# Serverless-Federated-Learning/FedLesScan

Hardware: AMD Instinct MI355X
Metric: aggregated GB/s (device-resident) — N-client FedAvg fp32 reduction (higher is better)
Workload: dtype f32

## Files before the change

### fedlesscan_amd/_lib.py

```python
from __future__ import annotations

import ctypes
import os
import re
import sysconfig
import threading

from .aggregator.exceptions import (
    AggregationError,
    InsufficientClientResults,
    InvalidParameterShapeError,
)

PKG = os.path.dirname(os.path.abspath(__file__))
REPO = os.path.dirname(PKG)
LIB_PATH = os.path.join(PKG, "_native", "libfedavg_hip.so")
BENCH_LIB_PATH = os.path.join(PKG, "_native", "libfedavg_hip_bench.so")
HOSTFAST_PATH = os.path.join(PKG, "_native", "_hostfast" + (sysconfig.get_config_var("EXT_SUFFIX") or ".so"))
HEADER = os.path.join(REPO, "include", "fedavg_hip.h")
BENCH_HEADER = os.path.join(REPO, "include", "fedavg_hip_bench.h")
ABI_VERSION = 7

FA_OK, FA_ERR_ARG, FA_ERR_NO_CLIENTS, FA_ERR_SHAPE, FA_ERR_HIP = range(5)

# ... 19 lines not shown
    "fa_finalize_f32": (_int, [_vp, _f32, _vp, _i64, _vp]),
    "fa_fedavg_bf16": (_int, [_vp, _i64, _i64, _i64, _vp, _vp, _f32, _vp, _vp, _vp]),
    "fa_fedavg_f16": (_int, [_vp, _i64, _i64, _i64, _vp, _vp, ctypes.c_uint16, _vp, _vp]),
    "fa_fold_f16": (_int, [_vp, _i64, _i64, _i64, _vp, _vp, _vp, ctypes.c_uint16, _int, _vp, _vp]),
    "fa_fedavg_bf16_ptrs": (_int, [_vp, _i64, _i64, _vp, _vp, _f32, _int, _vp, _vp, _vp]),
    "fa_fedavg_bf16_ptrs_hostf": (_int, [_vp, _i64, _i64, _vp, _vp, _f32, _int, _vp, _vp, _vp]),
    "fa_fedavg_f16_ptrs": (_int, [_vp, _i64, _i64, _vp, _vp, ctypes.c_uint16, _int, _vp, _vp]),
    "fa_rounds_create": (_int, [_vp, _int]),
    "fa_rounds_destroy": (_int, [_vp]),
    "fa_fedavg_f32_rounds": (_int, [_vp, _vp, _i64, _i64, _vp, _vp, _f32, _vp, _int, _vp, _vp, _vp]),
    "fa_fedavg_bf16_rounds": (_int, [_vp, _vp, _i64, _i64, _vp, _vp, _f32, _vp, _vp, _int, _vp, _vp, _vp]),
    "fa_fedavg_f32_rounds_hostf": (_int, [_vp, _vp, _i64, _i64, _vp, _vp, _f32, _vp, _int, _vp, _vp, _vp]),
    "fa_fedavg_bf16_rounds_hostf": (_int, [_vp, _vp, _i64, _i64, _vp, _vp, _f32, _vp, _vp, _int, _vp, _vp, _vp]),
    "fa_rounds_wait": (_int, [_vp, _int, _vp]),
    "fa_rounds_check": (_int, [_vp]),
    "fa_rounds_timeouts": (_int, [_vp]),
    "fa_rounds_form": (ctypes.c_char_p, [_int]),
    "fa_fedavg_f16_rounds": (_int, [_vp, _vp, _i64, _i64, _vp, _vp, ctypes.c_uint16, _vp, _int, _vp, _vp, _vp]),
    "fa_rounds_form_f16": (ctypes.c_char_p, []),
    "fa_fedavg_f64_rounds": (_int, [_vp, _vp, _i64, _i64, _vp, _vp, _f64, _vp, _int, _vp, _vp, _vp]),
    "fa_rounds_form_f64": (ctypes.c_char_p, []),
    "fa_peers_create": (_int, [_vp, _int, _int, _int, _i64]),
    "fa_peers_destroy": (_int, [_vp]),
    "fa_peers_handle_bytes": (_int, []),
    "fa_peers_handle": (_int, [_vp, _vp]),
    "fa_peers_open": (_int, [_vp, _vp]),
    "fa_peers_send": (_vp, [_vp]),
    "fa_peers_rounds": (_vp, [_vp]),
    "fa_peers_exchange": (_int, [_vp, _int, _vp, _vp, _vp, _vp]),
    "fa_fedavg_f64": (_int, [_vp, _i64, _i64, _i64, _vp, _vp, _f64, _vp, _vp]),
    "fa_fold_f64": (_int, [_vp, _i64, _i64, _i64, _vp, _vp, _vp, _f64, _int, _vp, _vp]),
    "fa_fedavg_f64_ptrs": (_int, [_vp, _i64, _i64, _vp, _vp, _f64, _int, _vp, _vp]),
    "fa_layers_plan": (_int, [_vp, _vp, _i64, _int, _i64, _int, _vp, _vp, _vp, _vp]),
    "fa_fedavg_f32_layers": (_int, [_vp, _vp, _i64, _i64, _i64, _int, _vp, _vp, _f32, _vp, _vp]),
    "fa_fedavg_bf16_layers": (_int, [_vp, _vp, _i64, _i64, _i64, _int, _vp, _vp, _f32, _vp, _vp, _vp]),
    "fa_fedavg_f16_layers": (_int, [_vp, _vp, _i64, _i64, _i64, _int, _vp, _vp, ctypes.c_uint16, _vp, _vp]),
    "fa_fedavg_f64_layers": (_int, [_vp, _vp, _i64, _i64, _i64, _int, _vp, _vp, _f64, _vp, _vp]),
    "fa_fedavg_i32": (_int, [_vp, _i64, _i64, _i64, _vp, _f64, _vp, _vp]),
    "fa_fedavg_i64": (_int, [_vp, _i64, _i64, _i64, _vp, _f64, _vp, _vp]),
    "fa_fedavg_i32_ptrs": (_int, [_vp, _i64, _i64, _vp, _vp, _f64, _int, _vp, _vp]),
    "fa_fedavg_i64_ptrs": (_int, [_vp, _i64, _i64, _vp, _vp, _f64, _int, _vp, _vp]),
    "fa_fedavg_i32_layers": (_int, [_vp, _vp, _i64, _i64, _i64, _int, _vp, _vp, _f64, _vp, _vp]),
    "fa_fedavg_i64_layers": (_int, [_vp, _vp, _i64, _i64, _i64, _int, _vp, _vp, _f64, _vp, _vp]),
    "fa_npz_index":(_int, [_vp, _i64, _vp, _vp, _vp, _vp, _vp, _int]),
    "fa_crc32": (_int, [_vp, _i64, ctypes.c_uint32, _int, ctypes.POINTER(ctypes.c_uint32)]),
    "fa_pack": (_int, [_vp, _vp, _vp, _vp, _i64, _int]),
    "fa_bson_elements": (_i64, [_vp, _i64, _i64, _vp, _vp, _vp, _vp, _vp, _vp, _i64]),
    "fa_bson_walk": (_i64, [_vp, _i64, _i64, _vp, _vp, _vp, _vp, _vp, _vp, _vp, _i64]),
    "fa_host_is_pinned": (_int, [_vp, _i64]),
    "fa_host_alloc": (_int, [_vp, _i64]),
    "fa_host_free": (_int, [_vp]),
    "fa_copy_h2d": (_int, [_vp, _vp, _i64, _vp]),
    "fa_copy_peer": (_int, [_vp, _int, _vp, _int, _i64, _vp]),
    "fa_set_autotune": (_int, [_int]),
    "fa_autotune_pending": (_int, []),
    "fa_fold_form": (ctypes.c_char_p, [_int, _i64, _i64, _i64, _int, _vp]),
    "fa_tune_cache_path": (_int, [ctypes.c_char_p]),
    "fa_tune_export": (_i64, [_vp, _i64]),
    "fa_tune_import": (_int, [ctypes.c_char_p]),
    "fa_step_lookup": (_int, [ctypes.c_char_p]),
    "fa_step_record": (_int, [ctypes.c_char_p, _int]),
    "fa_ingest_create": (_int, [_vp, _i64, _i64, _int, _int]),
    "fa_ingest_rows_per_chunk": (_int, [_vp]),
    "fa_ingest_begin": (_int, [_vp, _vp, _vp, _i64]),
    "fa_ingest_add": (_int, [_vp, _vp, _vp, _i64, _f32, _f32, _int]),
    "fa_ingest_finish": (_int, [_vp, _f32]),
# ... 149 lines not shown
```

### fedlesscan_amd/csrc/fedavg.hip

```cpp
#include "fold_kernels.hpp"
#include "peer_exchange.hpp"

#include <mutex>

namespace {

constexpr int kFactorSlots = 8;
struct FactorSlot {
    float* host = nullptr;
    float* dev = nullptr;
    size_t cap = 0;
    hipEvent_t ready = nullptr;
    hipEvent_t done = nullptr;
    bool pending = false;
};
struct FactorRing {
    std::mutex mu;
    FactorSlot slot[kFactorSlots];
    int next = 0;
    hipStream_t stage = nullptr;
};
FactorRing g_factor_rings[16];

constexpr int kFillFloats = 256;
// ... 407 lines not shown
    hipStream_t st = (hipStream_t)stream;
    StreamDevice on_stream_device(stream);
    if (aligned16(X) && aligned16(out) && (ldx % 2 == 0)) {
        if (s)
            hipLaunchKernelGGL((k_fedavg_f64_v2<8, true>), grid_for((P >> 1) + 1), dim3(kBlock), 0, st, X, N, P,
                               ldx, a, s, divisor, out);
        else
            hipLaunchKernelGGL((k_fedavg_f64_v2<8, false>), grid_for((P >> 1) + 1), dim3(kBlock), 0, st, X, N, P,
                               ldx, a, s, divisor, out);
        return check_launch("k_fedavg_f64_v2");
    }
    if (s)
        hipLaunchKernelGGL(k_fedavg_f64<true>, grid_for(P), dim3(kBlock), 0, st, X, N, P, ldx, a, s, divisor,
                           out);
    else
        hipLaunchKernelGGL(k_fedavg_f64<false>, grid_for(P), dim3(kBlock), 0, st, X, N, P, ldx, a, s, divisor,
                           out);
    return check_launch("k_fedavg_f64");
}

int fa_fold_f64(const double* X, int64_t N, int64_t P, int64_t ldx, const double* a, const double* s,
                const double* acc_in, double divisor, int finalize, double* out, void* stream) {
    return f64_fold(X, N, P, ldx, a, s, acc_in, divisor, finalize, out, stream);
}

int fa_fedavg_f64_ptrs(const double* const* xi, int64_t N, int64_t P, const double* a, const double* s,
                       double divisor, int rows_aligned, double* out, void* stream) {
    return f64_rows_fold(xi, N, P, a, s, divisor, rows_aligned, out, stream);
}

int fa_layers_plan(const int64_t* cols, const int32_t* aligned, int64_t L, int unit_lg, int64_t cus, int units,
                   fa_layer_plan* plan, int64_t* tiles, int64_t* elems, int* units_out) {
    return layers_plan(cols, aligned, L, unit_lg, cus, units, plan, tiles, elems, units_out);
}

int fa_fedavg_f32_layers(const float* const* xi, const fa_layer_plan* plan, int64_t L, int64_t N, int64_t tiles,
                         int units, const float* a, const float* s, float divisor, float* out, void* stream) {
    return layers_fold(kLayersF32, "fa_fedavg_f32_layers", (const void* const*)xi, plan, L, N, tiles, units, 0, a, s,
                       (double)divisor, out, nullptr, stream);
}

int fa_fedavg_bf16_layers(const uint16_t* const* xi, const fa_layer_plan* plan, int64_t L, int64_t N, int64_t tiles,
                          int units, const float* a, const float* s, float divisor, float* out_f32,
                          uint16_t* out_bf16, void* stream) {
    return layers_fold(kLayersBf16, "fa_fedavg_bf16_layers", (const void* const*)xi, plan, L, N, tiles, units, 0, a, s,
                       (double)divisor, out_f32, out_bf16, stream);
}

int fa_fedavg_f16_layers(const uint16_t* const* xi, const fa_layer_plan* plan, int64_t L, int64_t N, int64_t tiles,
                         int units, const uint16_t* a, const uint16_t* s, uint16_t divisor, uint16_t* out,
                         void* stream) {
    return layers_fold(kLayersF16, "fa_fedavg_f16_layers", (const void* const*)xi, plan, L, N, tiles, units, 0, a, s,
                       (double)half_bits_to_float(divisor), out, nullptr, stream);
}

int fa_fedavg_f64_layers(const double* const* xi, const fa_layer_plan* plan, int64_t L, int64_t N, int64_t tiles,
                         int units, const double* a, const double* s, double divisor, double* out, void* stream) {
    return layers_fold(kLayersF64, "fa_fedavg_f64_layers", (const void* const*)xi, plan, L, N, tiles, units, 0, a, s,
                       divisor, out, nullptr, stream);
}

int fa_fedavg_i32(const int32_t* X, int64_t N, int64_t P, int64_t ldx, const int64_t* a, double divisor,
                  double* out, void* stream) {
    int rc = check_common(N, P, ldx, X, a, out);
    if (rc) return rc;
    if (P == 0) { g_err[0] = 0; return FA_OK; }
// ... 183 lines not shown
```

### fedlesscan_amd/csrc/fold_kernels.hpp

```cpp
#pragma once
#include <hip/hip_runtime.h>
#include <stdarg.h>
#include <stdint.h>
#include <stdio.h>
#include <stdlib.h>
#include <string.h>

#include <atomic>
#include <map>
#include <mutex>
#include <string>
#include <tuple>
#include <type_traits>
#include <vector>

#include "fedavg_hip.h"
#include "octet_grid.hpp"
#include "layer_plan.hpp"
#include "tuner.hpp"

#pragma clang fp contract(off)

namespace {

// ... 1992 lines not shown
    for (; i < N; ++i) acc = acc + term1<SCORED>(((const gf32*)xi[i])[c], a[i], SCORED ? s[i] : 1.0f);
    return acc / divisor;
}

template <int U, int C, bool SCORED>
__global__ __launch_bounds__(kBlock) void k_fold_f32_layers(
    const float* const* __restrict__ xi, const fa_layer_plan* __restrict__ plan, int64_t L, int64_t N,
    const float* __restrict__ a, const float* __restrict__ s, float divisor, float* __restrict__ out,
    int64_t ntiles) {
    int64_t l = 0;
    for (int64_t bid = blockIdx.x; bid < ntiles; bid += gridDim.x) {
        const LayerTile t = layer_tile(plan, L, bid, l);
        l = t.l;
        const float* const* x = xi + l * N;
        float* o = out + t.offset;
        if (!t.aligned) {
            const int64_t c = t.bid * kBlock + threadIdx.x;
            if (c < t.cols) o[c] = fold_column_f32<SCORED>(x, c, N, a, s, divisor);
            continue;
        }
        f32x4* O4 = reinterpret_cast<f32x4*>(o);
        octet_tile<C, kBlock, 2>(
            t.bid, t.cols,
            [&](int64_t q) { fold_quads_rows<U, C, SCORED, gf32x4>(x, q, N, a, s, divisor, O4 + q); },
            [&](int64_t q) { fold_quads_rows<U, 1, SCORED, gf32x4>(x, q, N, a, s, divisor, O4 + q); },
            [&](int64_t col) {
                for (; col < t.cols; ++col) {
                    float acc = term1<SCORED>(((const gf32*)x[0])[col], a[0], SCORED ? s[0] : 1.0f);
                    for (int64_t i = 1; i < N; ++i)
                        acc = acc + term1<SCORED>(((const gf32*)x[i])[col], a[i], SCORED ? s[i] : 1.0f);
                    o[col] = acc / divisor;
                }
            });
    }
}

template <int U, int C, bool SCORED>
__global__ __launch_bounds__(kBlock) void k_fedavg_bf16_layers(
    const uint16_t* const* __restrict__ xi, const fa_layer_plan* __restrict__ plan, int64_t L, int64_t N,
    const float* __restrict__ a, const float* __restrict__ s, float divisor, float* __restrict__ out,
    uint16_t* __restrict__ outb, int64_t ntiles) {
    int64_t l = 0;
    for (int64_t bid = blockIdx.x; bid < ntiles; bid += gridDim.x) {
        const LayerTile t = layer_tile(plan, L, bid, l);
        l = t.l;
        const uint16_t* const* x = xi + l * N;
        float* o = out ? out + t.offset : nullptr;
        uint16_t* ob = outb ? outb + t.offset : nullptr;
        if (!t.aligned) {
            const int64_t c = t.bid * kBlock + threadIdx.x;
            if (c < t.cols) st_column_bf16(fold_column_bf16<SCORED>(TableRows<gu16>{x, c}, N, a, s, divisor), o, ob, c);
            continue;
        }
        octet_tile<C>(
            t.bid, t.cols,
            [&](int64_t q) { fold_octets<U, C, SCORED>(TableRows<gu32x4>{x, q}, N, a, s, divisor, o, ob, q); },
            [&](int64_t q) { fold_octets<U, 1, SCORED>(TableRows<gu32x4>{x, q}, N, a, s, divisor, o, ob, q); },
            [&](int64_t col) {
                for (; col < t.cols; ++col)
                    st_column_bf16(fold_column_bf16<SCORED>(TableRows<gu16>{x, col}, N, a, s, divisor), o, ob, col);
            });
    }
}

template <class A, int U, int C, bool SCORED>
__device__ __forceinline__ void native_layers(const typename A::E* const* __restrict__ xi,
// ... 1481 lines not shown
    switch (kind) {
        case kLayersF32: {
            const float* const* x = (const float* const*)xi;
            const float *af = (const float*)a, *sf = (const float*)s;
            if (s) FA_LAY(k_fold_f32_layers, true, x, plan, L, N, af, sf, (float)divisor, (float*)out);
            else FA_LAY(k_fold_f32_layers, false, x, plan, L, N, af, sf, (float)divisor, (float*)out);
            break;
        }
        case kLayersBf16: {
            const uint16_t* const* x = (const uint16_t* const*)xi;
            const float *af = (const float*)a, *sf = (const float*)s;
            if (s) FA_LAY(k_fedavg_bf16_layers, true, x, plan, L, N, af, sf, (float)divisor, (float*)out, (uint16_t*)outb);
            else FA_LAY(k_fedavg_bf16_layers, false, x, plan, L, N, af, sf, (float)divisor, (float*)out, (uint16_t*)outb);
            break;
        }
        case kLayersF16: {
            const uint16_t* const* x = (const uint16_t* const*)xi;
            const uint16_t *ah = (const uint16_t*)a, *sh = (const uint16_t*)s;
            if (s) FA_LAY(k_fedavg_f16_layers, true, x, plan, L, N, ah, sh, (float)divisor, (uint16_t*)out);
            else FA_LAY(k_fedavg_f16_layers, false, x, plan, L, N, ah, sh, (float)divisor, (uint16_t*)out);
            break;
        }
        default: {
            const double* const* x = (const double* const*)xi;
            const double *ad = (const double*)a, *sd = (const double*)s;
            if (s) FA_LAY(k_fedavg_f64_layers, true, x, plan, L, N, ad, sd, divisor, (double*)out);
            else FA_LAY(k_fedavg_f64_layers, false, x, plan, L, N, ad, sd, divisor, (double*)out);
            break;
        }
    }
#undef FA_LAY
}

inline int layers_fold(int kind, const char* what, const void* const* xi, const fa_layer_plan* plan, int64_t L,
                       int64_t N, int64_t tiles, int units, int64_t grid_cap, const void* a, const void* s,
                       double divisor, void* out, void* outb, void* stream) {
    if (kind < kLayersF32 || kind > kLayersF64) return fail(FA_ERR_ARG, "%s: unknown dtype %d", what, kind);
    if (L < 0 || N < 0 || tiles < 0)
        return fail(FA_ERR_ARG, "negative size (L=%lld, N=%lld, tiles=%lld)", (long long)L, (long long)N,
                    (long long)tiles);
    if (N == 0) return fail(FA_ERR_NO_CLIENTS, "no client results to aggregate (N == 0)");
    if (units != 1 && units != 2 && units != 4)
        return fail(FA_ERR_ARG, "%s: %d units per lane (1, 2 or 4)", what, units);
    if (grid_cap < 0) return fail(FA_ERR_ARG, "%s: negative grid cap", what);
    if (L == 0 || tiles == 0) { g_err[0] = 0; return FA_OK; }
    const bool any_out = kind == kLayersBf16 ? (out || outb) : out != nullptr;
    if (!xi || !plan || !a || !any_out) return fail(FA_ERR_ARG, "null xi/plan/a/out pointer");
    if (!aligned16(out) || (kind == kLayersBf16 && !aligned16(outb)))
        return fail(FA_ERR_ARG, "%s needs 16-B aligned outputs", what);
    if (tiles > (int64_t)0x7FFFFFFF) return fail(FA_ERR_ARG, "too many tiles for one launch");
    hipStream_t st = (hipStream_t)stream;
    StreamDevice on_stream_device(stream);
    int64_t g = tile_grid(tiles, -1, cu_count());
    if (grid_cap > 0 && g > grid_cap) g = grid_cap;
    if (kind != kLayersBf16) outb = nullptr;
    switch (units) {
        case 4: launch_layers<4>(kind, st, (unsigned)g, xi, plan, L, N, tiles, a, s, divisor, out, outb); break;
        case 2: launch_layers<2>(kind, st, (unsigned)g, xi, plan, L, N, tiles, a, s, divisor, out, outb); break;
        default: launch_layers<1>(kind, st, (unsigned)g, xi, plan, L, N, tiles, a, s, divisor, out, outb); break;
    }
    return check_launch(what);
}

template <class I, int C>
void launch_int_layers(hipStream_t st, unsigned g, const typename I::T* const* xi, const fa_layer_plan* plan,
                       const fa_layer_plan& one, int64_t L, int64_t N, int64_t tiles, const int64_t* a, const double* s,
                       double divisor, double* out) {
    if (s)
        hipLaunchKernelGGL((k_fedavg_int_layers<I, kLayersU, C, true>), dim3(g), dim3(kBlock), 0, st, xi, plan, one, L,
                           N, a, s, divisor, out, tiles);
    else
        hipLaunchKernelGGL((k_fedavg_int_layers<I, kLayersU, C, false>), dim3(g), dim3(kBlock), 0, st, xi, plan, one, L,
                           N, a, s, divisor, out, tiles);
}

template <class I>
void launch_int_layers_units(int units, hipStream_t st, unsigned g, const typename I::T* const* xi,
                             const fa_layer_plan* plan, const fa_layer_plan& one, int64_t L, int64_t N, int64_t tiles,
                             const int64_t* a, const double* s, double divisor, double* out) {
    switch (units) {
        case 4: launch_int_layers<I, 4>(st, g, xi, plan, one, L, N, tiles, a, s, divisor, out); break;
        case 2: launch_int_layers<I, 2>(st, g, xi, plan, one, L, N, tiles, a, s, divisor, out); break;
        default: launch_int_layers<I, 1>(st, g, xi, plan, one, L, N, tiles, a, s, divisor, out); break;
    }
}
// ... 18 lines not shown
    int64_t g = tile_grid(tiles, -1, cu_count());
    if (grid_cap > 0 && g > grid_cap) g = grid_cap;
    launch_int_layers_units<I>(units, st, (unsigned)g, xi, plan, fa_layer_plan{0, 0, 0, 0}, L, N, tiles, a, s, divisor,
                               out);
    return check_launch(what);
}

template <class I>
int int_rows_fold(const char* what, const typename I::T* const* xi, int64_t N, int64_t P, const int64_t* a,
                  const double* s, double divisor, int rows_aligned, double* out, void* stream) {
    int rc = check_common(N, P, P, xi, a, out);
    if (rc) return rc;
    if (P == 0) { g_err[0] = 0; return FA_OK; }
    if (rows_aligned && !aligned16(out))
        return fail(FA_ERR_ARG, "the unit form of the integer row-table fold needs 16-B aligned rows and out");
    hipStream_t st = (hipStream_t)stream;
    StreamDevice on_stream_device(stream);
    const int64_t cus = cu_count();
    const int32_t al = rows_aligned != 0;
    const int units = pick_layer_units(&P, &al, 1, I::LG, cus);
    fa_layer_plan one;
    int64_t elems = 0;
    const int64_t tiles = fill_layer_plan(&P, &al, 1, units, I::LG, &one, &elems);
    if (tiles > (int64_t)0x7FFFFFFF) return fail(FA_ERR_ARG, "too many tiles for one launch");
    launch_int_layers_units<I>(units, st, (unsigned)tile_grid(tiles, -1, cus), xi, nullptr, one, 1, N, tiles, a, s,
                               divisor, out);
    return check_launch(what);
}

inline int layers_plan(const int64_t* cols, const int32_t* aligned, int64_t L, int unit_lg, int64_t cus, int units,
                       fa_layer_plan* plan, int64_t* tiles, int64_t* elems, int* units_out) {
    if (L < 0 || cus < 1 || unit_lg < 1 || unit_lg > 3)
        return fail(FA_ERR_ARG, "fa_layers_plan: L=%lld, cus=%lld, unit_lg=%d", (long long)L, (long long)cus, unit_lg);
    if (units != 0 && units != 1 && units != 2 && units != 4)
        return fail(FA_ERR_ARG, "fa_layers_plan: %d units per lane (0, 1, 2 or 4)", units);
    if (!tiles || !elems || !units_out || (L > 0 && (!cols || !aligned || !plan)))
        return fail(FA_ERR_ARG, "fa_layers_plan: null pointer");
    for (int64_t l = 0; l < L; ++l)
        if (cols[l] < 0) return fail(FA_ERR_ARG, "fa_layers_plan: layer %lld has %lld columns", (long long)l,
                                     (long long)cols[l]);
    if (units == 0) units = pick_layer_units(cols, aligned, L, unit_lg, cus);
    *tiles = fill_layer_plan(cols, aligned, L, units, unit_lg, plan, elems);
    *units_out = units;
    g_err[0] = 0;
    return FA_OK;
}

}
```

### fedlesscan_amd/csrc/layer_plan.hpp

```cpp
#pragma once
#include <stdint.h>

#include "fedavg_hip.h"
#include "octet_grid.hpp"

constexpr int64_t kLayerOutAlign = 64;

inline int64_t layer_tiles(int64_t cols, bool aligned, int units, int unit_lg) {
    if (cols <= 0) return 0;
    if (!aligned) return (cols + kBlock - 1) / kBlock;
    return octet_grid(cols, units, 0, 1, unit_lg).tiles;
}

inline int64_t layers_total_tiles(const int64_t* cols, const int32_t* aligned, int64_t L, int units, int unit_lg) {
    int64_t t = 0;
    for (int64_t l = 0; l < L; ++l) t += layer_tiles(cols[l], aligned[l] != 0, units, unit_lg);
    return t;
}

inline int pick_layer_units(const int64_t* cols, const int32_t* aligned, int64_t L, int unit_lg, int64_t cus) {
    for (int c = 4; c > 1; c >>= 1)
        if (tile_grid(layers_total_tiles(cols, aligned, L, c, unit_lg), -1, cus) * 8 >= cus * 7) return c;
    return 1;
}

inline int64_t fill_layer_plan(const int64_t* cols, const int32_t* aligned, int64_t L, int units, int unit_lg,
                               fa_layer_plan* plan, int64_t* elems) {
    int64_t t = 0, off = 0;
    for (int64_t l = 0; l < L; ++l) {
        plan[l].cols = cols[l];
        plan[l].offset = off;
        plan[l].tile0 = t;
        plan[l].aligned = aligned[l] != 0;
        t += layer_tiles(cols[l], aligned[l] != 0, units, unit_lg);
        off += (cols[l] + kLayerOutAlign - 1) / kLayerOutAlign * kLayerOutAlign;
    }
    *elems = off;
    return t;
}
```

### fedlesscan_amd/engine.py

```python
from __future__ import annotations

import ctypes
import functools
import operator
import os
import threading
from typing import List, NamedTuple, Optional, Sequence

import numpy as np
import torch

from . import _lib
from .aggregator.exceptions import InvalidParameterShapeError

_TORCH_TO_NP = {torch.float32: np.float32, torch.float64: np.float64, torch.int32: np.int32,
                torch.int64: np.int64, torch.float16: np.float16}
_NP_TO_TORCH = {np.dtype(np.float32): torch.float32, np.dtype(np.float64): torch.float64,
                np.dtype(np.int32): torch.int32, np.dtype(np.int64): torch.int64,
                np.dtype(np.float16): torch.float16}
ROW_ALIGN = 64


def default_device() -> torch.device:
    if not torch.cuda.is_available():
# ... 656 lines not shown
        a, s = f.to(dev)
        _lib.call("fa_fedavg_f64_rounds", r, X.data_ptr(), N, ldx, a.data_ptr(), _ptr(s), float(f.div),
                  addr(out), rounds, offs, oo, st)
    else:
        raise InvalidParameterShapeError(
            f"the rounds fold takes float32, bfloat16, float16 or float64 rows, got {X.dtype}")
    return r


def wait_round(state: ctypes.c_void_p, k: int, stream: torch.cuda.Stream) -> None:
    _lib.call("fa_rounds_wait", state, int(k), stream.cuda_stream)


def _equal_stride_view(rows, host_ptrs: np.ndarray, P: int) -> Optional[torch.Tensor]:
    N = len(rows)
    if N < 2 or P == 0:
        return None
    esize = rows[0].element_size()
    step = int(host_ptrs[1] - host_ptrs[0])
    if step < P * esize or step % esize:
        return None
    if (np.diff(host_ptrs) != step).any():
        return None
    base, last = rows[0], rows[-1]
    if last.untyped_storage().data_ptr() != base.untyped_storage().data_ptr():
        return None
    return base.as_strided((N, P), (step // esize, 1))


_dtype_of = operator.attrgetter("dtype")
_ROW_TABLE_DTYPES = (torch.float32, torch.bfloat16, torch.float16, torch.float64, torch.int32, torch.int64)
_INT_ROWS = {torch.int32: "fa_fedavg_i32_ptrs", torch.int64: "fa_fedavg_i64_ptrs"}
_NO_CAPTURE_TABLE = (torch.float64, torch.int32, torch.int64)
stats = {"rows16_folds": 0, "rows64_folds": 0, "stacked_groups": 0, "layer_table_folds": 0, "rows_int_folds": 0}


class RowSet:

    def __init__(self, rows: Sequence[torch.Tensor]):
        rows = list(rows)
        N = len(rows)
        if N == 0:
            _lib.check(_lib.FA_ERR_NO_CLIENTS, "RowSet")
        r0 = rows[0]
        P, dev, dt = r0.numel(), r0.device, r0.dtype
        if not r0.is_cuda:
            raise ValueError("rows must be CUDA (HIP) tensors")
        if (set(map(torch.Tensor.numel, rows)) != {P} or set(map(_dtype_of, rows)) != {dt}
                or not all(map(torch.Tensor.is_contiguous, rows))
                or set(map(torch.Tensor.get_device, rows)) != {r0.get_device()}):
            raise InvalidParameterShapeError("all rows must be contiguous with equal size, dtype, device")
        self.rows = rows
        self.N, self.P, self.device, self.dtype = N, P, dev, dt
        self.view = None
        self.ptrs = None
        self.host_ptrs = None
        self.aligned = False
        if dt in _ROW_TABLE_DTYPES and P > 0 and not (dt in _NO_CAPTURE_TABLE
                                                      and torch.cuda.is_current_stream_capturing()):
            host_ptrs = self.host_ptrs = np.fromiter(map(torch.Tensor.data_ptr, rows), dtype=np.int64, count=N)
            self.view = _equal_stride_view(rows, host_ptrs, P)
            if self.view is None:
                self.ptrs = torch.from_numpy(host_ptrs).to(dev)
                self.aligned = not (host_ptrs % 16).any()

    def overlaps(self, t: torch.Tensor) -> bool:
        if self.host_ptrs is None or self.P == 0 or t.numel() == 0:
# ... 165 lines not shown


_LAYER_TABLE = {
    torch.float32: ("fa_fedavg_f32_layers", 2),
    torch.bfloat16: ("fa_fedavg_bf16_layers", 3),
    torch.float16: ("fa_fedavg_f16_layers", 3),
    torch.float64: ("fa_fedavg_f64_layers", 1),
    torch.int32: ("fa_fedavg_i32_layers", 2),
    torch.int64: ("fa_fedavg_i64_layers", 1),
}
_shape_of = operator.attrgetter("shape")
_cu_counts: dict = {}


def _cus(dev: torch.device) -> int:
    k = dev.index if dev.index is not None else torch.cuda.current_device()
    n = _cu_counts.get(k)
    if n is None:
        n = _cu_counts[k] = int(torch.cuda.get_device_properties(k).multi_processor_count)
    return n


def layer_plan(cols: Sequence[int], aligned: Sequence[bool], unit_lg: int, cus: int, units: int = 0):
    L = len(cols)
    c = np.ascontiguousarray(cols, dtype=np.int64)
    al = np.ascontiguousarray(aligned, dtype=np.int32)
    plan = np.zeros((L, 4), dtype=np.int64)
    tiles, elems, u = ctypes.c_int64(), ctypes.c_int64(), ctypes.c_int()
    _lib.call("fa_layers_plan", c.ctypes.data, al.ctypes.data, L, unit_lg, cus, units, plan.ctypes.data,
              ctypes.addressof(tiles), ctypes.addressof(elems), ctypes.addressof(u))
    return plan, tiles.value, elems.value, u.value


class ModelRowSet:

    def __init__(self, parameters: Sequence[Sequence[torch.Tensor]], layers: Optional[Sequence[int]] = None):
        params = list(parameters)
        N = len(params)
        if N == 0:
            _lib.check(_lib.FA_ERR_NO_CLIENTS, "ModelRowSet")
        lis = list(range(min(map(len, params)))) if layers is None else list(layers)
        cols_of = [list(map(operator.itemgetter(li), params)) for li in lis]
        t0 = cols_of[0][0] if cols_of else None
        if t0 is not None and not (isinstance(t0, torch.Tensor) and t0.is_cuda):
            raise ValueError("layers must be CUDA (HIP) tensors")
        self.N, self.L, self.layers = N, len(lis), lis
        self.device = t0.device if t0 is not None else None
        self.dtype = t0.dtype if t0 is not None else None
        self.shapes, self.sizes = [], []
        host_ptrs = np.zeros((self.L, N), dtype=np.int64)
        for k, col in enumerate(cols_of):
            shp = col[0].shape
            if (set(map(_shape_of, col)) != {shp} or set(map(_dtype_of, col)) != {self.dtype}
                    or not all(map(torch.Tensor.is_contiguous, col))
                    or set(map(torch.Tensor.get_device, col)) != {t0.get_device()}):
                raise InvalidParameterShapeError(
                    f"layer {lis[k]}: all clients' tensors must be contiguous with one shape, dtype and device")
            self.shapes.append(tuple(shp))
            self.sizes.append(col[0].numel())
            host_ptrs[k] = np.fromiter(map(torch.Tensor.data_ptr, col), dtype=np.int64, count=N)
        self.tensors = cols_of
        self.host_ptrs = host_ptrs
        self.esize = t0.element_size() if t0 is not None else 0
        self.entry = None
        self._rowsets: dict = {}
        self.ptrs = self.plan = self.host_plan = None
        self.tiles = self.elems = self.units = 0
        if self.dtype in _LAYER_TABLE and self.L:
            self.entry, lg = _LAYER_TABLE[self.dtype]
            sizes = np.asarray(self.sizes, dtype=np.int64)
            aligned = ~((host_ptrs % 16) != 0).any(axis=1) | (sizes == 0)
            self.host_plan, self.tiles, self.elems, self.units = layer_plan(sizes, aligned, lg, _cus(self.device))
            both = torch.from_numpy(np.concatenate([host_ptrs.reshape(-1), self.host_plan.reshape(-1)])).to(self.device)
            self.ptrs, self.plan = both[:self.L * N], both[self.L * N:]
        self.offsets = [int(o) for o in self.host_plan[:, 1]] if self.host_plan is not None else []

    def overlaps(self, t: torch.Tensor) -> bool:
        if self.L == 0 or t.numel() == 0:
            return False
        lo = t.data_ptr()
        hi = lo + t.numel() * t.element_size()
        nbytes = (np.asarray(self.sizes, dtype=np.int64) * self.esize)[:, None]
        return bool(np.any((self.host_ptrs < hi) & (lo < self.host_ptrs + nbytes)))

    def rowset(self, k: int) -> RowSet:
        rs = self._rowsets.get(k)
        if rs is None:
            rows = [t.reshape(-1) for t in self.tensors[k]]
            if self.ptrs is None or self.sizes[k] == 0:
                rs = RowSet(rows)
            else:
                rs = RowSet.__new__(RowSet)
                rs.rows, rs.N, rs.P, rs.device, rs.dtype = rows, self.N, self.sizes[k], self.device, self.dtype
                rs.view = None
                rs.ptrs = self.ptrs[k * self.N:(k + 1) * self.N]
                rs.host_ptrs = self.host_ptrs[k]
                rs.aligned = bool(self.host_plan[k, 3])
            self._rowsets[k] = rs
        return rs

    def split(self, flat: torch.Tensor) -> List[torch.Tensor]:
        return [flat[o:o + n].reshape(s) for o, n, s in zip(self.offsets, self.sizes, self.shapes)]


def layer_table_enabled() -> bool:
    return os.environ.get("FEDAVG_LAYER_TABLE", "1") != "0"

# ... 18 lines not shown
    if len(weights) != N or (scores is not None and len(scores) != N):
        raise InvalidParameterShapeError(f"{N} clients but {len(weights)} weights"
                                         + ("" if scores is None else f" / {len(scores)} scores"))
    bf16 = ms.dtype == torch.bfloat16
    if (out_bf16 is not None or want_bf16) and not bf16:
        raise InvalidParameterShapeError("want_bf16 / out_bf16 are for bfloat16 layers")
    f = None
    if ms.entry is not None and not torch.cuda.is_current_stream_capturing():
        f = _layer_factors(ms.dtype, weights, scores, total)
    if f is None:
        if out is not None or out_bf16 is not None:
            raise InvalidParameterShapeError("out / out_bf16 need the layer-table route (no promotion, no capture)")
        res = [fold_rows(ms.rowset(k), weights, scores, total=total, want_bf16=want_bf16) for k in range(ms.L)]
        if want_bf16:
            return ([r[0].reshape(s) for r, s in zip(res, ms.shapes)],
                    [r[1].reshape(s) for r, s in zip(res, ms.shapes)])
        return [r.reshape(s) for r, s in zip(res, ms.shapes)]
    dev, E = ms.device, ms.elems
    res_dt = torch.float32 if bf16 else torch.float64 if ms.dtype in _INT_ROWS else ms.dtype
    _check_out("out", out, res_dt, E)
    _check_out("out_bf16", out_bf16, torch.bfloat16, E)

    def usable(t):
        return t is not None and t.data_ptr() % 16 == 0 and not ms.overlaps(t)

    dst, dstb = out, out_bf16
    out = out if usable(out) else None
    outb = out_bf16 if usable(out_bf16) else None
    if outb is None and (want_bf16 or dstb is not None):
        outb = torch.empty(E, dtype=torch.bfloat16, device=dev)
    if out is None and (dst is not None or outb is None or want_bf16):
        out = torch.empty(E, dtype=res_dt, device=dev)
    a, s = f.to(dev)
    args = [ms.ptrs.data_ptr(), ms.plan.data_ptr(), ms.L, N, ms.tiles, ms.units, a.data_ptr(), _ptr(s)]
    if bf16:
        _lib.call(ms.entry, *args, float(f.div), _ptr(out), _ptr(outb), stream_ptr(dev))
    elif ms.dtype == torch.float16:
        _lib.call(ms.entry, *args, _half_bits(f.div), out.data_ptr(), stream_ptr(dev))
    else:
        _lib.call(ms.entry, *args, float(f.div), out.data_ptr(), stream_ptr(dev))
    stats["layer_table_folds"] += 1
    folded = sum(1 for n in ms.sizes if n)
    if ms.dtype == torch.float64:
        stats["rows64_folds"] += folded
    elif ms.dtype in _INT_ROWS:
        stats["rows_int_folds"] += folded
    elif ms.dtype != torch.float32:
        stats["rows16_folds"] += folded
    if dst is not None and dst is not out:
        dst.reshape(-1)[:E].copy_(out)
        out = dst
    if dstb is not None and dstb is not outb:
        dstb.reshape(-1)[:E].copy_(outb)
        outb = dstb
    if want_bf16:
        return ms.split(out.reshape(-1)), ms.split(outb.reshape(-1))
    if out_bf16 is not None:
        return ms.split(outb.reshape(-1)) if out is None else (ms.split(out.reshape(-1)), ms.split(outb.reshape(-1)))
    return ms.split(out.reshape(-1))


def _layer_meta(parameters, n_eff):
    L = min(len(p) for p in parameters[:n_eff])
    shapes, dtypes = [], []
    for li in range(L):
        ref = parameters[0][li]
        shp = tuple(ref.shape)
        dt, mixed = ref.dtype, False
        for ci in range(1, n_eff):
            x = parameters[ci][li]
            if tuple(x.shape) != shp:
                raise InvalidParameterShapeError(
                    f"layer {li}: client {ci} has shape {tuple(x.shape)}, client 0 has {shp}")
            mixed = mixed or x.dtype != dt
# ... 247 lines not shown
```

### include/fedavg_hip.h

```cpp
#ifndef FEDAVG_HIP_H
#define FEDAVG_HIP_H

#include <stdint.h>

#ifdef __cplusplus
extern "C" {
#endif

#define FA_ABI_VERSION 7

enum fa_status {
    FA_OK = 0,
    FA_ERR_ARG = 1,
    FA_ERR_NO_CLIENTS = 2,
    FA_ERR_SHAPE = 3,
    FA_ERR_HIP = 4,
};

int fa_abi_version(void);
const char* fa_last_error(void);

int fa_fedavg_f32(const float* X, int64_t N, int64_t P, int64_t ldx,
                  const float* a, const float* s, float divisor,
                  float* out, void* stream);
// ... 97 lines not shown
    FA_FOLD_BF16 = 2,
    FA_FOLD_F32_ROWS = 3,
    FA_FOLD_F16 = 4,
};
int fa_set_autotune(int mode);
int fa_autotune_pending(void);
const char* fa_fold_form(int kind, int64_t N, int64_t P, int64_t ldx, int scored, void* stream);
int fa_tune_cache_path(const char* path);
int64_t fa_tune_export(char* buf, int64_t cap);
int fa_tune_import(const char* text);
int fa_step_lookup(const char* key);
int fa_step_record(const char* key, int one_launch);

int fa_fedavg_f64(const double* X, int64_t N, int64_t P, int64_t ldx,
                  const double* a, const double* s, double divisor,
                  double* out, void* stream);

int fa_fold_f64(const double* X, int64_t N, int64_t P, int64_t ldx,
                const double* a, const double* s, const double* acc_in,
                double divisor, int finalize, double* out, void* stream);

int fa_fedavg_f64_ptrs(const double* const* xi, int64_t N, int64_t P,
                       const double* a, const double* s, double divisor, int rows_aligned,
                       double* out, void* stream);

typedef struct fa_layer_plan {
    int64_t cols;
    int64_t offset;
    int64_t tile0;
    int64_t aligned;
} fa_layer_plan;
int fa_layers_plan(const int64_t* cols, const int32_t* aligned, int64_t L, int unit_lg, int64_t cus, int units,
                   fa_layer_plan* plan, int64_t* tiles, int64_t* elems, int* units_out);
int fa_fedavg_f32_layers(const float* const* xi, const fa_layer_plan* plan, int64_t L, int64_t N, int64_t tiles,
                         int units, const float* a, const float* s, float divisor, float* out, void* stream);
int fa_fedavg_bf16_layers(const uint16_t* const* xi, const fa_layer_plan* plan, int64_t L, int64_t N, int64_t tiles,
                          int units, const float* a, const float* s, float divisor, float* out_f32,
                          uint16_t* out_bf16, void* stream);
int fa_fedavg_f16_layers(const uint16_t* const* xi, const fa_layer_plan* plan, int64_t L, int64_t N, int64_t tiles,
                         int units, const uint16_t* a, const uint16_t* s, uint16_t divisor, uint16_t* out,
                         void* stream);
int fa_fedavg_f64_layers(const double* const* xi, const fa_layer_plan* plan, int64_t L, int64_t N, int64_t tiles,
                         int units, const double* a, const double* s, double divisor, double* out, void* stream);

int fa_fedavg_i32(const int32_t* X, int64_t N, int64_t P, int64_t ldx,
                  const int64_t* a, double divisor, double* out, void* stream);
int fa_fedavg_i64(const int64_t* X, int64_t N, int64_t P, int64_t ldx,
                  const int64_t* a, double divisor, double* out, void* stream);

int fa_fedavg_i32_ptrs(const int32_t* const* xi, int64_t N, int64_t P, const int64_t* a, const double* s,
                       double divisor, int rows_aligned, double* out, void* stream);
int fa_fedavg_i64_ptrs(const int64_t* const* xi, int64_t N, int64_t P, const int64_t* a, const double* s,
                       double divisor, int rows_aligned, double* out, void* stream);
int fa_fedavg_i32_layers(const int32_t* const* xi, const fa_layer_plan* plan, int64_t L, int64_t N, int64_t tiles,
                         int units, const int64_t* a, const double* s, double divisor, double* out, void* stream);
int fa_fedavg_i64_layers(const int64_t* const* xi, const fa_layer_plan* plan, int64_t L, int64_t N, int64_t tiles,
                         int units, const int64_t* a, const double* s, double divisor, double* out, void* stream);

int fa_host_is_pinned(const void* p, int64_t n);
int fa_host_alloc(void** p, int64_t n);
int fa_host_free(void* p);
int fa_copy_h2d(void* dst, const void* src, int64_t n, void* stream);

int fa_copy_peer(void* dst, int dst_device, const void* src, int src_device, int64_t n, void* stream);

typedef struct fa_ingest fa_ingest;
// ... 39 lines not shown
```

Before: 7100.

## Add LDS-staged row-tile kernel for f32 layer-table FedAvg folds

```diff
diff --git a/fedlesscan_amd/_lib.py b/fedlesscan_amd/_lib.py
--- a/fedlesscan_amd/_lib.py
+++ b/fedlesscan_amd/_lib.py
@@ -75,6 +75,7 @@
     "fa_fold_f64": (_int, [_vp, _i64, _i64, _i64, _vp, _vp, _vp, _f64, _int, _vp, _vp]),
     "fa_fedavg_f64_ptrs": (_int, [_vp, _i64, _i64, _vp, _vp, _f64, _int, _vp, _vp]),
     "fa_layers_plan": (_int, [_vp, _vp, _i64, _int, _i64, _int, _vp, _vp, _vp, _vp]),
+    "fa_layers_pick_f32": (_int, [_vp, _vp, _i64, _i64, _i64, _vp]),
     "fa_fedavg_f32_layers": (_int, [_vp, _vp, _i64, _i64, _i64, _int, _vp, _vp, _f32, _vp, _vp]),
     "fa_fedavg_bf16_layers": (_int, [_vp, _vp, _i64, _i64, _i64, _int, _vp, _vp, _f32, _vp, _vp, _vp]),
     "fa_fedavg_f16_layers": (_int, [_vp, _vp, _i64, _i64, _i64, _int, _vp, _vp, ctypes.c_uint16, _vp, _vp]),
diff --git a/fedlesscan_amd/csrc/fedavg.hip b/fedlesscan_amd/csrc/fedavg.hip
--- a/fedlesscan_amd/csrc/fedavg.hip
+++ b/fedlesscan_amd/csrc/fedavg.hip
@@ -463,6 +463,11 @@
 int fa_layers_plan(const int64_t* cols, const int32_t* aligned, int64_t L, int unit_lg, int64_t cus, int units,
                    fa_layer_plan* plan, int64_t* tiles, int64_t* elems, int* units_out) {
     return layers_plan(cols, aligned, L, unit_lg, cus, units, plan, tiles, elems, units_out);
+}
+
+int fa_layers_pick_f32(const int64_t* cols, const int32_t* aligned, int64_t L, int64_t N, int64_t cus,
+                       int* units_out) {
+    return layers_pick_f32(cols, aligned, L, N, cus, units_out);
 }
 
 int fa_fedavg_f32_layers(const float* const* xi, const fa_layer_plan* plan, int64_t L, int64_t N, int64_t tiles,
diff --git a/fedlesscan_amd/csrc/fold_kernels.hpp b/fedlesscan_amd/csrc/fold_kernels.hpp
--- a/fedlesscan_amd/csrc/fold_kernels.hpp
+++ b/fedlesscan_amd/csrc/fold_kernels.hpp
@@ -2048,6 +2048,208 @@
                     o[col] = acc / divisor;
                 }
             });
+    }
+}
+
+template <int NW, int R, int TQ, bool SCORED, int DEPTH>
+__device__ __forceinline__ void lds_rows_tile(int64_t bid, const float* const* __restrict__ xi, int64_t N, int64_t P,
+                                              const float* __restrict__ a, const float* __restrict__ s, float divisor,
+                                              float* __restrict__ out, f32x4* tile, float* fa, float* fs) {
+    constexpr int NT = NW * 64;
+    constexpr int LQ = R * TQ / NT;
+    static_assert(TQ <= 64 && (R * TQ) % NT == 0 && R <= NT, "tile shape");
+    const int64_t nq = P >> 2;
+    const int64_t nbq = (nq + TQ - 1) / TQ;
+    const int t = threadIdx.x;
+
+    if (bid >= nbq) {
+        const int w4 = (int)(P & 3);
+        const int64_t col0 = nq * 4;
+        f32x4 acc = {0.f, 0.f, 0.f, 0.f};
+        for (int64_t r0 = 0; r0 < N; r0 += NT) {
+            const int64_t row = r0 + t;
+            if (row < N) {
+                const gf32* rp = (const gf32*)xi[row];
+                f32x4 x = {0.f, 0.f, 0.f, 0.f};
+                for (int k = 0; k < w4; ++k) x[k] = rp[col0 + k];
+                tile[t] = term4<SCORED>(x, a[row], SCORED ? s[row] : 1.0f);
+            }
+            __syncthreads();
+            if (t == 0) {
+                const int rows = (N - r0) < NT ? (int)(N - r0) : NT;
+                int i = 0;
+                if (r0 == 0) {
+                    acc = tile[0];
+                    i = 1;
+                }
+                for (; i + 8 <= rows; i += 8) {
+                    f32x4 v[8];
+#pragma unroll
+                    for (int k = 0; k < 8; ++k) v[k] = tile[i + k];
+#pragma unroll
+                    for (int k = 0; k < 8; ++k) acc = add4(acc, v[k]);
+                }
+                for (; i < rows; ++i) acc = add4(acc, tile[i]);
+            }
+            __syncthreads();
+        }
+        if (t == 0) {
+            const f32x4 res = div4(acc, divisor);
+            for (int k = 0; k < w4; ++k) out[col0 + k] = res[k];
+        }
+        return;
+    }
+
+    const int64_t q0 = bid * TQ;
+    const int tq = (int)((nq - q0) < TQ ? (nq - q0) : TQ);
+    auto qof = [&](int j) -> int64_t {
+        const int64_t q = q0 + (t + j * NT) % TQ;
+        return q < nq ? q : nq - 1;
+    };
+    struct Stage {
+        f32x4 v[LQ];
+        float fv, sv;
+    };
+    Stage st[DEPTH > 1 ? DEPTH : 1];
+    const int64_t nfull = N / R;
+    const float* nxt[LQ];
+    auto fetch_ptrs = [&](int64_t c) {
+        const int64_t cc = c < nfull ? c : nfull - 1;
+#pragma unroll
+        for (int j = 0; j < LQ; ++j) nxt[j] = xi[cc * R + (t + j * NT) / TQ];
+    };
+    auto load_full = [&](int64_t c, Stage& g) {
+#pragma unroll
+        for (int j = 0; j < LQ; ++j) g.v[j] = __builtin_nontemporal_load((const gf32x4*)nxt[j] + qof(j));
+        if (t < R) {
+            g.fv = a[c * R + t];
+            if constexpr (SCORED) g.sv = s[c * R + t];
+        }
+        if (c + 1 < nfull) fetch_ptrs(c + 1);
+    };
+    auto load_rows_checked = [&](int64_t c, Stage& g) {
+#pragma unroll
+        for (int j = 0; j < LQ; ++j) {
+            const int64_t row = c * R + (t + j * NT) / TQ;
+            if (row < N) g.v[j] = __builtin_nontemporal_load((const gf32x4*)xi[row] + qof(j));
+        }
+        if (t < R && c * R + t < N) {
+            g.fv = a[c * R + t];
+            if constexpr (SCORED) g.sv = s[c * R + t];
+        }
+    };
+    auto stash = [&](const Stage& g) {
+#pragma unroll
+        for (int j = 0; j < LQ; ++j) tile[t + j * NT] = g.v[j];
+        if (t < R) {
+            fa[t] = g.fv;
+            if constexpr (SCORED) fs[t] = g.sv;
+        }
+    };
+    constexpr int TC = TQ * 4, CPW = (TC + NW - 1) / NW;
+    static_assert(CPW <= 64, "column fold: at most one column per lane");
+    const int ccol = (t >> 6) * CPW + (t & 63);
+    const bool cfold = (t & 63) < CPW && ccol < tq * 4;
+    const float* tilef = reinterpret_cast<const float*>(tile);
+    float acc1 = 0.f;
+    auto fold = [&](int64_t c, int rows) {
+        if (cfold) {
+            int r = 0;
+            if (c == 0) {
+                acc1 = term1<SCORED>(tilef[ccol], fa[0], SCORED ? fs[0] : 1.0f);
+                r = 1;
+            }
+            for (; r + 8 <= rows; r += 8) {
+                float x[8], f[8], g[8];
+#pragma unroll
+                for (int k = 0; k < 8; ++k) {
+                    x[k] = tilef[(r + k) * TC + ccol];
+                    f[k] = fa[r + k];
+                    g[k] = SCORED ? fs[r + k] : 1.0f;
+                }
+#pragma unroll
+                for (int k = 0; k < 8; ++k) acc1 = acc1 + term1<SCORED>(x[k], f[k], g[k]);
+            }
+            for (; r < rows; ++r) acc1 = acc1 + term1<SCORED>(tilef[r * TC + ccol], fa[r], SCORED ? fs[r] : 1.0f);
+        }
+    };
+    int64_t c = 0;
+    if (DEPTH >= 2 && nfull > DEPTH) {
+        fetch_ptrs(0);
+        load_full(0, st[0]);
+        stash(st[0]);
+        __syncthreads();
+#pragma unroll
+        for (int k = 1; k <= DEPTH; ++k) load_full(k, st[k % DEPTH]);
+        for (; c + 2 * DEPTH < nfull; c += DEPTH) {
+#pragma unroll
+            for (int k = 0; k < DEPTH; ++k) {
+                fold(c + k, R);
+                __syncthreads();
+                stash(st[(k + 1) % DEPTH]);
+                __syncthreads();
+                load_full(c + k + 1 + DEPTH, st[(k + 1) % DEPTH]);
+            }
+        }
+#pragma unroll
+        for (int k = 0; k < 2 * DEPTH; ++k) {
+            const int64_t cc = c + k;
+            if (cc < nfull) {
+                fold(cc, R);
+                __syncthreads();
+                if (cc + 1 < nfull) {
+                    stash(st[(k + 1) % DEPTH]);
+                    __syncthreads();
+                    if (cc + 1 + DEPTH < nfull) load_full(cc + 1 + DEPTH, st[(k + 1) % DEPTH]);
+                }
+            }
+        }
+        c = nfull;
+    } else if (nfull > 0) {
+        fetch_ptrs(0);
+        load_full(0, st[0]);
+        stash(st[0]);
+        __syncthreads();
+        for (; c + 1 < nfull; ++c) {
+            load_full(c + 1, st[0]);
+            fold(c, R);
+            __syncthreads();
+            stash(st[0]);
+            __syncthreads();
+        }
+        fold(c, R);
+        __syncthreads();
+        ++c;
+    }
+    if (c * R < N) {
+        load_rows_checked(c, st[0]);
+        stash(st[0]);
+        __syncthreads();
+        fold(c, (int)(N - c * R));
+        __syncthreads();
+    }
+    if (cfold) __builtin_nontemporal_store(acc1 / divisor, out + q0 * 4 + ccol);
+}
+
+template <int NW, int R, int TQ, int DEPTH, bool SCORED>
+__global__ __launch_bounds__(NW * 64) void k_fold_f32_layers_lds(
+    const float* const* __restrict__ xi, const fa_layer_plan* __restrict__ plan, int64_t L, int64_t N,
+    const float* __restrict__ a, const float* __restrict__ s, float divisor, float* __restrict__ out,
+    int64_t ntiles) {
+    __shared__ f32x4 tile[R * TQ];
+    __shared__ float fa[R], fs[SCORED ? R : 1];
+    int64_t l = 0;
+    for (int64_t bid = blockIdx.x; bid < ntiles; bid += gridDim.x) {
+        const LayerTile t = layer_tile(plan, L, bid, l);
+        l = t.l;
+        const float* const* x = xi + l * N;
+        float* o = out + t.offset;
+        if (!t.aligned) {
+            const int64_t c = t.bid * (NW * 64) + threadIdx.x;
+            if (c < t.cols) o[c] = fold_column_f32<SCORED>(x, c, N, a, s, divisor);
+            continue;
+        }
+        lds_rows_tile<NW, R, TQ, SCORED, DEPTH>(t.bid, x, N, t.cols, a, s, divisor, o, tile, fa, fs);
     }
 }
 
@@ -3595,6 +3797,45 @@
 #undef FA_LAY
 }
 
+template <int F>
+void launch_layers_lds_form(hipStream_t st, unsigned g, const float* const* xi, const fa_layer_plan* plan, int64_t L,
+                            int64_t N, int64_t tiles, const float* a, const float* s, float divisor, float* out) {
+    constexpr LayersLdsForm f = kLayersLdsForms[F];
+    if (s)
+        hipLaunchKernelGGL((k_fold_f32_layers_lds<f.nw, f.r, f.tq, f.depth, true>), dim3(g), dim3(f.nw * 64), 0, st, xi,
+                           plan, L, N, a, s, divisor, out, tiles);
+    else
+        hipLaunchKernelGGL((k_fold_f32_layers_lds<f.nw, f.r, f.tq, f.depth, false>), dim3(g), dim3(f.nw * 64), 0, st,
+                           xi, plan, L, N, a, s, divisor, out, tiles);
+}
+inline void launch_layers_lds(int f, hipStream_t st, unsigned g, const float* const* xi, const fa_layer_plan* plan,
+                              int64_t L, int64_t N, int64_t tiles, const float* a, const float* s, float divisor,
+                              float* out) {
+    switch (f) {
+        case kLayW2T16D2: launch_layers_lds_form<kLayW2T16D2>(st, g, xi, plan, L, N, tiles, a, s, divisor, out); break;
+        case kLayW2T32: launch_layers_lds_form<kLayW2T32>(st, g, xi, plan, L, N, tiles, a, s, divisor, out); break;
+        case kLayW4T24: launch_layers_lds_form<kLayW4T24>(st, g, xi, plan, L, N, tiles, a, s, divisor, out); break;
+        case kLayW4T40: launch_layers_lds_form<kLayW4T40>(st, g, xi, plan, L, N, tiles, a, s, divisor, out); break;
+        case kLayW8: launch_layers_lds_form<kLayW8>(st, g, xi, plan, L, N, tiles, a, s, divisor, out); break;
+        default: launch_layers_lds_form<kLayW4T32>(st, g, xi, plan, L, N, tiles, a, s, divisor, out); break;
+    }
+}
+
+inline int pick_layers_lds(const int64_t* cols, const int32_t* aligned, int64_t L, int64_t N, int64_t cus) {
+    int64_t P = 0;
+    for (int64_t l = 0; l < L; ++l)
+        if (aligned[l] && cols[l] > 0) P += cols[l];
+    const int64_t nq = P >> 2;
+    if (nq < 1 || nq >= ((int64_t)3 << 18)) return 0;
+    if (nq >= 20480) return kLayersLds + kLayW2T32;
+    switch (pick_f32(N, P, cus)) {
+        case F32Pick::kLdsW4T24: return kLayersLds + kLayW4T24;
+        case F32Pick::kLdsW4T40: return kLayersLds + kLayW4T40;
+        default: break;
+    }
+    return kLayersLds + kLayW2T16D2;
+}
+
 inline int layers_fold(int kind, const char* what, const void* const* xi, const fa_layer_plan* plan, int64_t L,
                        int64_t N, int64_t tiles, int units, int64_t grid_cap, const void* a, const void* s,
                        double divisor, void* out, void* outb, void* stream) {
@@ -3603,7 +3844,8 @@
         return fail(FA_ERR_ARG, "negative size (L=%lld, N=%lld, tiles=%lld)", (long long)L, (long long)N,
                     (long long)tiles);
     if (N == 0) return fail(FA_ERR_NO_CLIENTS, "no client results to aggregate (N == 0)");
-    if (units != 1 && units != 2 && units != 4)
+    const bool lds = kind == kLayersF32 && layers_lds_units(units);
+    if (units != 1 && units != 2 && units != 4 && !lds)
         return fail(FA_ERR_ARG, "%s: %d units per lane (1, 2 or 4)", what, units);
     if (grid_cap < 0) return fail(FA_ERR_ARG, "%s: negative grid cap", what);
     if (L == 0 || tiles == 0) { g_err[0] = 0; return FA_OK; }
@@ -3614,6 +3856,12 @@
     if (tiles > (int64_t)0x7FFFFFFF) return fail(FA_ERR_ARG, "too many tiles for one launch");
     hipStream_t st = (hipStream_t)stream;
     StreamDevice on_stream_device(stream);
+    if (lds) {
+        launch_layers_lds(units - kLayersLds, st, (unsigned)(grid_cap > 0 && tiles > grid_cap ? grid_cap : tiles),
+                          (const float* const*)xi, plan, L, N, tiles, (const float*)a, (const float*)s, (float)divisor,
+                          (float*)out);
+        return check_launch(what);
+    }
     int64_t g = tile_grid(tiles, -1, cu_count());
     if (grid_cap > 0 && g > grid_cap) g = grid_cap;
     if (kind != kLayersBf16) outb = nullptr;
@@ -3698,7 +3946,7 @@
                        fa_layer_plan* plan, int64_t* tiles, int64_t* elems, int* units_out) {
     if (L < 0 || cus < 1 || unit_lg < 1 || unit_lg > 3)
         return fail(FA_ERR_ARG, "fa_layers_plan: L=%lld, cus=%lld, unit_lg=%d", (long long)L, (long long)cus, unit_lg);
-    if (units != 0 && units != 1 && units != 2 && units != 4)
+    if (units != 0 && units != 1 && units != 2 && units != 4 && !(unit_lg == 2 && layers_lds_units(units)))
         return fail(FA_ERR_ARG, "fa_layers_plan: %d units per lane (0, 1, 2 or 4)", units);
     if (!tiles || !elems || !units_out || (L > 0 && (!cols || !aligned || !plan)))
         return fail(FA_ERR_ARG, "fa_layers_plan: null pointer");
@@ -3712,4 +3960,18 @@
     return FA_OK;
 }
 
-}
+inline int layers_pick_f32(const int64_t* cols, const int32_t* aligned, int64_t L, int64_t N, int64_t cus,
+                           int* units_out) {
+    if (L < 0 || N < 1 || cus < 1)
+        return fail(FA_ERR_ARG, "fa_layers_pick_f32: L=%lld, N=%lld, cus=%lld", (long long)L, (long long)N,
+                    (long long)cus);
+    if (!units_out || (L > 0 && (!cols || !aligned))) return fail(FA_ERR_ARG, "fa_layers_pick_f32: null pointer");
+    for (int64_t l = 0; l < L; ++l)
+        if (cols[l] < 0) return fail(FA_ERR_ARG, "fa_layers_pick_f32: layer %lld has %lld columns", (long long)l,
+                                     (long long)cols[l]);
+    *units_out = pick_layers_lds(cols, aligned, L, N, cus);
+    g_err[0] = 0;
+    return FA_OK;
+}
+
+}
diff --git a/fedlesscan_amd/csrc/layer_plan.hpp b/fedlesscan_amd/csrc/layer_plan.hpp
--- a/fedlesscan_amd/csrc/layer_plan.hpp
+++ b/fedlesscan_amd/csrc/layer_plan.hpp
@@ -6,8 +6,27 @@
 
 constexpr int64_t kLayerOutAlign = 64;
 
+struct LayersLdsForm {
+    const char* name;
+    int nw, r, tq, depth;
+};
+constexpr int kLayersLds = 16;
+constexpr LayersLdsForm kLayersLdsForms[] = {
+    {"layers_lds_w2_t16_d2", 2, 32, 16, 2}, {"layers_lds_w2_t32", 2, 16, 32, 2}, {"layers_lds_w4_t24", 4, 32, 24, 2},
+    {"layers_lds_w4_t40", 4, 32, 40, 2},    {"layers_lds_w8_t32", 8, 64, 32, 1}, {"layers_lds_w4_t32", 4, 16, 32, 2},
+};
+constexpr int kNumLayersLdsForms = (int)(sizeof(kLayersLdsForms) / sizeof(kLayersLdsForms[0]));
+static_assert(kLayersLds == FA_LAYERS_LDS && kNumLayersLdsForms == FA_LAYERS_LDS_FORMS, "the header's values");
+enum LayersLdsIndex { kLayW2T16D2 = 0, kLayW2T32, kLayW4T24, kLayW4T40, kLayW8, kLayW4T32 };
+inline bool layers_lds_units(int units) { return units >= kLayersLds && units < kLayersLds + kNumLayersLdsForms; }
+
 inline int64_t layer_tiles(int64_t cols, bool aligned, int units, int unit_lg) {
     if (cols <= 0) return 0;
+    if (layers_lds_units(units)) {
+        const LayersLdsForm& f = kLayersLdsForms[units - kLayersLds];
+        if (!aligned) return (cols + f.nw * 64 - 1) / (f.nw * 64);
+        return ((cols >> 2) + f.tq - 1) / f.tq + ((cols & 3) ? 1 : 0);
+    }
     if (!aligned) return (cols + kBlock - 1) / kBlock;
     return octet_grid(cols, units, 0, 1, unit_lg).tiles;
 }
diff --git a/fedlesscan_amd/engine.py b/fedlesscan_amd/engine.py
--- a/fedlesscan_amd/engine.py
+++ b/fedlesscan_amd/engine.py
@@ -712,7 +712,8 @@
 _ROW_TABLE_DTYPES = (torch.float32, torch.bfloat16, torch.float16, torch.float64, torch.int32, torch.int64)
 _INT_ROWS = {torch.int32: "fa_fedavg_i32_ptrs", torch.int64: "fa_fedavg_i64_ptrs"}
 _NO_CAPTURE_TABLE = (torch.float64, torch.int32, torch.int64)
-stats = {"rows16_folds": 0, "rows64_folds": 0, "stacked_groups": 0, "layer_table_folds": 0, "rows_int_folds": 0}
+stats = {"rows16_folds": 0, "rows64_folds": 0, "stacked_groups": 0, "layer_table_folds": 0, "rows_int_folds": 0,
+         "layer_lds_folds": 0}
 
 
 class RowSet:
@@ -944,6 +945,21 @@
     return plan, tiles.value, elems.value, u.value
 
 
+LAYERS_LDS = 16
+
+
+def layer_pick_f32(cols: Sequence[int], aligned: Sequence[bool], clients: int, cus: int) -> int:
+    c = np.ascontiguousarray(cols, dtype=np.int64)
+    al = np.ascontiguousarray(aligned, dtype=np.int32)
+    u = ctypes.c_int()
+    _lib.call("fa_layers_pick_f32", c.ctypes.data, al.ctypes.data, len(cols), clients, cus, ctypes.addressof(u))
+    return u.value
+
+
+def layer_lds_enabled() -> bool:
+    return os.environ.get("FEDAVG_LAYER_LDS", "1") != "0"
+
+
 class ModelRowSet:
 
     def __init__(self, parameters: Sequence[Sequence[torch.Tensor]], layers: Optional[Sequence[int]] = None):
@@ -978,13 +994,24 @@
         self._rowsets: dict = {}
         self.ptrs = self.plan = self.host_plan = None
         self.tiles = self.elems = self.units = 0
+        self.lds_units = self.lds_tiles = 0
+        self.lds_plan = self.lds_host_plan = None
         if self.dtype in _LAYER_TABLE and self.L:
             self.entry, lg = _LAYER_TABLE[self.dtype]
             sizes = np.asarray(self.sizes, dtype=np.int64)
             aligned = ~((host_ptrs % 16) != 0).any(axis=1) | (sizes == 0)
-            self.host_plan, self.tiles, self.elems, self.units = layer_plan(sizes, aligned, lg, _cus(self.device))
-            both = torch.from_numpy(np.concatenate([host_ptrs.reshape(-1), self.host_plan.reshape(-1)])).to(self.device)
-            self.ptrs, self.plan = both[:self.L * N], both[self.L * N:]
+            cus = _cus(self.device)
+            self.host_plan, self.tiles, self.elems, self.units = layer_plan(sizes, aligned, lg, cus)
+            parts = [host_ptrs.reshape(-1), self.host_plan.reshape(-1)]
+            if self.dtype == torch.float32:
+                self.lds_units = layer_pick_f32(sizes, aligned, N, cus)
+            if self.lds_units:
+                self.lds_host_plan, self.lds_tiles, _, _ = layer_plan(sizes, aligned, lg, cus, self.lds_units)
+                parts.append(self.lds_host_plan.reshape(-1))
+            both = torch.from_numpy(np.concatenate(parts)).to(self.device)
+            self.ptrs, self.plan = both[:self.L * N], both[self.L * N:self.L * (N + 4)]
+            if self.lds_units:
+                self.lds_plan = both[self.L * (N + 4):]
         self.offsets = [int(o) for o in self.host_plan[:, 1]] if self.host_plan is not None else []
 
     def overlaps(self, t: torch.Tensor) -> bool:
@@ -1069,7 +1096,11 @@
     if out is None and (dst is not None or outb is None or want_bf16):
         out = torch.empty(E, dtype=res_dt, device=dev)
     a, s = f.to(dev)
-    args = [ms.ptrs.data_ptr(), ms.plan.data_ptr(), ms.L, N, ms.tiles, ms.units, a.data_ptr(), _ptr(s)]
+    lds = bool(ms.lds_units) and layer_lds_enabled()
+    if lds:
+        args = [ms.ptrs.data_ptr(), ms.lds_plan.data_ptr(), ms.L, N, ms.lds_tiles, ms.lds_units, a.data_ptr(), _ptr(s)]
+    else:
+        args = [ms.ptrs.data_ptr(), ms.plan.data_ptr(), ms.L, N, ms.tiles, ms.units, a.data_ptr(), _ptr(s)]
     if bf16:
         _lib.call(ms.entry, *args, float(f.div), _ptr(out), _ptr(outb), stream_ptr(dev))
     elif ms.dtype == torch.float16:
@@ -1077,6 +1108,7 @@
     else:
         _lib.call(ms.entry, *args, float(f.div), out.data_ptr(), stream_ptr(dev))
     stats["layer_table_folds"] += 1
+    stats["layer_lds_folds"] += lds
     folded = sum(1 for n in ms.sizes if n)
     if ms.dtype == torch.float64:
         stats["rows64_folds"] += folded
diff --git a/include/fedavg_hip.h b/include/fedavg_hip.h
--- a/include/fedavg_hip.h
+++ b/include/fedavg_hip.h
@@ -153,6 +153,10 @@
 } fa_layer_plan;
 int fa_layers_plan(const int64_t* cols, const int32_t* aligned, int64_t L, int unit_lg, int64_t cus, int units,
                    fa_layer_plan* plan, int64_t* tiles, int64_t* elems, int* units_out);
+#define FA_LAYERS_LDS 16
+#define FA_LAYERS_LDS_FORMS 6
+int fa_layers_pick_f32(const int64_t* cols, const int32_t* aligned, int64_t L, int64_t N, int64_t cus,
+                       int* units_out);
 int fa_fedavg_f32_layers(const float* const* xi, const fa_layer_plan* plan, int64_t L, int64_t N, int64_t tiles,
                          int units, const float* a, const float* s, float divisor, float* out, void* stream);
 int fa_fedavg_bf16_layers(const uint16_t* const* xi, const fa_layer_plan* plan, int64_t L, int64_t N, int64_t tiles,
```

Result: no change. 7101 (median of 2 runs) (+0.0%).
